# Bitcoin-Wildlife-Sanctuary/recursive-stwo

Measured on AMD Instinct MI355X. Metric: recursive proofs verified/sec, higher is better.
Workload: dtype u32 (M31 modular integers)

## Files before the change

### recursive-stwo_amd/csrc/poseidon2.hpp

```cpp
#pragma once
#include "field.hpp"

namespace rsv {

struct State16 {
    uint32_t s[16];
};

#define RSV_RC_FULL_INIT { \
    {0x768bab52, 0x70e0ab7d, 0x3d266c8a, 0x6da42045, 0x600fef22, 0x41dace6b, 0x64f9bdd4, 0x5d42d4fe, \
     0x76b1516d, 0x6fc9a717, 0x70ac4fb6, 0x00194ef6, 0x22b644e2, 0x1f7916d5, 0x47581be2, 0x2710a123}, \
    {0x6284e867, 0x018d3afe, 0x5df99ef3, 0x4c1e467b, 0x566f6abc, 0x2994e427, 0x538a6d42, 0x5d7bf2cf, \
     0x7fda2dab, 0x0fd854c4, 0x46922fca, 0x3d7763a1, 0x19fd05ca, 0x0a4bbb43, 0x15075851, 0x3d903d76}, \
    {0x2d290ff7, 0x40809fa0, 0x59dac6ec, 0x127927a2, 0x6bbf0ea0, 0x0294140f, 0x24742976, 0x6e84c081, \
     0x22484f4a, 0x354cae59, 0x0453ffe1, 0x3f47a3cc, 0x0088204e, 0x6066e109, 0x3b7c4b80, 0x6b55665d}, \
    {0x3bc4b897, 0x735bf378, 0x508daf42, 0x1884fc2b, 0x7214f24c, 0x7498be0a, 0x1a60e640, 0x3303f928, \
     0x29b46376, 0x5c96bb68, 0x65d097a5, 0x1d358e9f, 0x4a9a9017, 0x4724cf76, 0x347af70f, 0x1e77e59a}, \
    {0x57090613, 0x1fa42108, 0x17bbef50, 0x1ff7e11c, 0x047b24ca, 0x4e140275, 0x4fa086f5, 0x079b309c, \
     0x1159bd47, 0x6d37e4e5, 0x075d8dce, 0x12121ca0, 0x7f6a7c40, 0x68e182ba, 0x5493201b, 0x0444a80e}, \
    {0x0064f4c6, 0x6467abe6, 0x66975762, 0x2af68f9b, 0x345b33be, 0x1b70d47f, 0x053db717, 0x381189cb, \
     0x43b915f8, 0x20df3694, 0x0f459d26, 0x77a0e97b, 0x2f73e739, 0x1876c2f9, 0x65a0e29a, 0x4cabefbe}, \
    {0x5abd1268, 0x4d34a760, 0x12771799, 0x69a0c9ac, 0x39091e55, 0x7f611cd0, 0x3af055da, 0x7ac0bbdf, \
     0x6e0f3a24, 0x41e3b6f7, 0x49b3756d, 0x568bc538, 0x20c079d8, 0x1701c72c, 0x7670dc6c, 0x5a439035}, \
    {0x7c93e00e, 0x561fbb4d, 0x1178907b, 0x02737406, 0x32fb24f1, 0x6323b60a, 0x6ab12418, 0x42c99cea, \
     0x155a0b97, 0x53d1c6aa, 0x2bd20347, 0x279b3d73, 0x4f5f3c70, 0x0245af6c, 0x238359d3, 0x49966a59}}
__constant__ __attribute__((aligned(64))) uint32_t RC_FULL[8][16] = RSV_RC_FULL_INIT;
constexpr uint32_t RC_FULL_K[8][16] = RSV_RC_FULL_INIT;

#define RSV_RC_PARTIAL_INIT { \
   0x7f7ec4bf, 0x0421926f, 0x5198e669, 0x34db3148, 0x4368bafd, \
                                        0x66685c7f, 0x78d3249a, 0x60187881, 0x76dad67a, 0x0690b437, \
                                        0x1ea95311, 0x40e5369a, 0x38f103fc, 0x1d226a21, 0, 0}
__constant__ __attribute__((aligned(64))) uint32_t RC_PARTIAL[16] = RSV_RC_PARTIAL_INIT;
constexpr uint32_t RC_PARTIAL_K[16] = RSV_RC_PARTIAL_INIT;

__device__ __forceinline__ uint32_t pow5_ref(uint32_t x) {
    uint32_t x2 = m_sqr(x);
    return m_mul(m_sqr(x2), x);
}

__device__ __forceinline__ void mds4_ref(uint32_t& x0, uint32_t& x1, uint32_t& x2, uint32_t& x3) {
    uint32_t t0 = m_add(x0, x1), t1 = m_add(x2, x3);
    uint32_t t2 = m_add(m_dbl(x1), t1), t3 = m_add(m_dbl(x3), t0);
    uint32_t t4 = m_add(m_shl(t1, 2), t3), t5 = m_add(m_shl(t0, 2), t2);
    x0 = m_add(t3, t5);
    x1 = t5;
    x2 = m_add(t2, t4);
    x3 = t4;
}

__device__ __forceinline__ void mds16_ref(uint32_t* s) {
#pragma unroll
    for (int g = 0; g < 4; g++) mds4_ref(s[4 * g], s[4 * g + 1], s[4 * g + 2], s[4 * g + 3]);
#pragma unroll
    for (int j = 0; j < 4; j++) {
        uint32_t sum = m_add(m_add(s[j], s[j + 4]), m_add(s[j + 8], s[j + 12]));
#pragma unroll
        for (int g = 0; g < 4; g++) s[4 * g + j] = m_add(s[4 * g + j], sum);
    }
}

__device__ __forceinline__ void poseidon2_ref_inline(uint32_t* s) {
    mds16_ref(s);
#pragma unroll 1
    for (int r = 0; r < 4; r++) {
#pragma unroll
        for (int i = 0; i < 16; i++) s[i] = pow5_ref(m_add(s[i], RC_FULL[r][i]));
        mds16_ref(s);
    }
#pragma unroll 1
    for (int r = 0; r < 14; r++) {
        s[0] = pow5_ref(m_add(s[0], RC_PARTIAL[r]));
        uint32_t a0 = m_add(s[0], s[1]), a1 = m_add(s[2], s[3]), a2 = m_add(s[4], s[5]), a3 = m_add(s[6], s[7]);
        uint32_t a4 = m_add(s[8], s[9]), a5 = m_add(s[10], s[11]), a6 = m_add(s[12], s[13]),
                 a7 = m_add(s[14], s[15]);
        uint32_t sum = m_add(m_add(m_add(a0, a1), m_add(a2, a3)), m_add(m_add(a4, a5), m_add(a6, a7)));
        s[0] = m_add(sum, m_add(m_dbl(s[0]), s[0]));
#pragma unroll
        for (int i = 1; i < 16; i++) s[i] = m_add(sum, m_shl(s[i], i + 1));
    }
#pragma unroll 1
    for (int r = 4; r < 8; r++) {
#pragma unroll
        for (int i = 0; i < 16; i++) s[i] = pow5_ref(m_add(s[i], RC_FULL[r][i]));
        mds16_ref(s);
    }
}


template <bool PACE>
struct PermT {
    static __device__ __forceinline__ uint64_t add64(uint64_t a, uint64_t b) {
        uint64_t d;
        asm("v_lshl_add_u64 %0, %1, 0, %2" : "=v"(d) : "v"(a), "v"(b));
        return d;
    }
    template <int SH>
    static __device__ __forceinline__ uint64_t shl_add64(uint64_t a, uint64_t b) {
        uint64_t d;
        asm("v_lshl_add_u64 %0, %1, %3, %2" : "=v"(d) : "v"(a), "v"(b), "n"(SH));
        return d;
    }
    static __device__ __forceinline__ uint32_t opaque(uint32_t k) {
        uint32_t r;
        asm volatile("s_mov_b32 %0, %1" : "=s"(r) : "n"(k));
        return r;
    }
    static __device__ __forceinline__ uint64_t mul64(uint32_t a, uint32_t b) {
        uint64_t d, carry;
        if constexpr (PACE) asm("v_mad_u64_u32 %0, %1, %2, %3, 0\n\ts_nop 0" : "=v"(d), "=s"(carry) : "v"(a), "v"(b));
        else asm("v_mad_u64_u32 %0, %1, %2, %3, 0" : "=v"(d), "=s"(carry) : "v"(a), "v"(b));
        return d;
    }
    static __device__ __forceinline__ uint64_t mul64(uint32_t a, uint32_t b_uniform, int) {
        uint64_t d, carry;
        if constexpr (PACE) asm("v_mad_u64_u32 %0, %1, %2, %3, 0\n\ts_nop 0" : "=v"(d), "=s"(carry) : "v"(a), "s"(b_uniform));
        else asm("v_mad_u64_u32 %0, %1, %2, %3, 0" : "=v"(d), "=s"(carry) : "v"(a), "s"(b_uniform));
        return d;
    }
    static __device__ __forceinline__ uint64_t mad64(uint32_t a, uint32_t b_uniform, uint64_t c) {
        uint64_t d, carry;
        if constexpr (PACE) asm("v_mad_u64_u32 %0, %1, %2, %3, %4\n\ts_nop 0" : "=v"(d), "=s"(carry) : "v"(a), "s"(b_uniform), "v"(c));
        else asm("v_mad_u64_u32 %0, %1, %2, %3, %4" : "=v"(d), "=s"(carry) : "v"(a), "s"(b_uniform), "v"(c));
        return d;
    }
    static __device__ __forceinline__ uint32_t dbl32(uint32_t x) {
        uint32_t d;
        asm("v_add_u32 %0, %1, %1" : "=v"(d) : "v"(x));
        return d;
    }
    static __device__ __forceinline__ uint32_t fold2(uint64_t V) {
        uint32_t r = (uint32_t)(V >> 32) + ((uint32_t)V >> 1);
        return r;
    }
    static __device__ __forceinline__ uint32_t canon(uint32_t t) {
        uint32_t r = min(t, t - P);
        if constexpr (PACE) asm volatile("s_nop 0" : "+v"(r));
        return r;
    }

    static __device__ __forceinline__ uint32_t pow5(uint32_t x) {
        const uint32_t xx = dbl32(x);
        uint32_t c2 = canon(fold2(mul64(xx, x)));
        uint32_t c4 = canon(fold2(mul64(dbl32(c2), c2)));
        return fold2(mul64(xx, c4));
    }

    static __device__ __forceinline__ void mds4_2x(uint32_t k2, uint32_t k4, uint32_t x0, uint32_t x1, uint32_t x2, uint32_t x3,
                                            uint64_t& y0, uint64_t& y1, uint64_t& y2, uint64_t& y3) {
        uint64_t T0 = mad64(x0, k2, mul64(x1, k2, 0));
        uint64_t T1 = mad64(x2, k2, mul64(x3, k2, 0));
        uint64_t T2 = mad64(x1, k4, T1);
        uint64_t T3 = mad64(x3, k4, T0);
        uint64_t T4 = shl_add64<2>(T1, T3);
        uint64_t T5 = shl_add64<2>(T0, T2);
        y0 = add64(T3, T5);
        y1 = T5;
        y2 = add64(T2, T4);
        y3 = T4;
    }

    static __device__ __forceinline__ void mds16_2x(uint32_t k2, uint32_t k4, const uint32_t* s, uint64_t* V) {
    #pragma unroll
        for (int g = 0; g < 4; g++)
            mds4_2x(k2, k4, s[4 * g], s[4 * g + 1], s[4 * g + 2], s[4 * g + 3], V[4 * g], V[4 * g + 1], V[4 * g + 2], V[4 * g + 3]);
    #pragma unroll
        for (int j = 0; j < 4; j++) {
            uint64_t sum = add64(add64(V[j], V[j + 4]), add64(V[j + 8], V[j + 12]));
    #pragma unroll
            for (int g = 0; g < 4; g++) V[4 * g + j] = add64(V[4 * g + j], sum);
        }
    }

    template <uint32_t RC>
    static __device__ __forceinline__ uint32_t canon_rc(uint32_t t) {
        static_assert(RC < P - (1u << 19), "round constant too close to P for the fused reduction");
        constexpr uint32_t c = P - RC;
        uint32_t r = min(t - c, t + (P - c));
        if constexpr (PACE) asm volatile("s_nop 0" : "+v"(r));
        return r;
    }

    template <int R, int I>
    static __device__ __forceinline__ void sbox_full(const uint64_t* V, uint32_t* s) {
        s[I] = pow5(canon_rc<RC_FULL_K[R][I]>(fold2(V[I])));
        if constexpr (I + 1 < 16) sbox_full<R, I + 1>(V, s);
    }
    template <int I>
    static __device__ __forceinline__ void sbox_full4(uint32_t* s) {
        s[I] = pow5(canon_rc<RC_FULL_K[4][I]>(s[I]));
        if constexpr (I + 1 < 16) sbox_full4<I + 1>(s);
    }

    template <int R>
    static __device__ __forceinline__ void partial_round(uint32_t* s, uint32_t k2, uint32_t k6, const uint32_t* kd) {
        uint32_t u0 = pow5(canon_rc<RC_PARTIAL_K[R]>(s[0]));
        uint64_t a = mul64(u0, k2, 0), b = mul64(s[1], k2, 0);
    #pragma unroll
        for (int i = 2; i < 16; i += 2) { a = mad64(s[i], k2, a); b = mad64(s[i + 1], k2, b); }
        uint64_t sum2 = add64(a, b);
        s[0] = fold2(mad64(u0, k6, sum2));
    #pragma unroll
        for (int i = 1; i < 16; i++) s[i] = fold2(mad64(s[i], kd[i], sum2));
    }

    static __device__ __forceinline__ void poseidon2_rounds(uint32_t* s, uint32_t k2, uint32_t k4) {
        uint64_t V[16];
        const uint32_t k6 = opaque(6);
        mds16_2x(k2, k4, s, V);
        sbox_full<0, 0>(V, s); mds16_2x(k2, k4, s, V);
        sbox_full<1, 0>(V, s); mds16_2x(k2, k4, s, V);
        sbox_full<2, 0>(V, s); mds16_2x(k2, k4, s, V);
        sbox_full<3, 0>(V, s); mds16_2x(k2, k4, s, V);
    #pragma unroll
        for (int i = 0; i < 16; i++) s[i] = fold2(V[i]);
        uint32_t kd[16];
        kd[0] = k6;
    #define RSV_KD(i) kd[i] = opaque(4u << (i));
        RSV_KD(1) RSV_KD(2) RSV_KD(3) RSV_KD(4) RSV_KD(5) RSV_KD(6) RSV_KD(7) RSV_KD(8)
        RSV_KD(9) RSV_KD(10) RSV_KD(11) RSV_KD(12) RSV_KD(13) RSV_KD(14) RSV_KD(15)
    #undef RSV_KD
        partial_round<0>(s, k2, k6, kd);  partial_round<1>(s, k2, k6, kd);  partial_round<2>(s, k2, k6, kd);
        partial_round<3>(s, k2, k6, kd);  partial_round<4>(s, k2, k6, kd);  partial_round<5>(s, k2, k6, kd);
        partial_round<6>(s, k2, k6, kd);  partial_round<7>(s, k2, k6, kd);  partial_round<8>(s, k2, k6, kd);
        partial_round<9>(s, k2, k6, kd);  partial_round<10>(s, k2, k6, kd); partial_round<11>(s, k2, k6, kd);
        partial_round<12>(s, k2, k6, kd); partial_round<13>(s, k2, k6, kd);
        sbox_full4<0>(s);      mds16_2x(k2, k4, s, V);
        sbox_full<5, 0>(V, s); mds16_2x(k2, k4, s, V);
        sbox_full<6, 0>(V, s); mds16_2x(k2, k4, s, V);
        sbox_full<7, 0>(V, s);
    }

    static __device__ __forceinline__ void poseidon2_inline(uint32_t* s) {
        const uint32_t k2 = opaque(2), k4 = opaque(4);
        poseidon2_rounds(s, k2, k4);
        uint64_t V[16];
        mds16_2x(k2, k4, s, V);
    #pragma unroll
        for (int i = 0; i < 16; i++) {
            uint32_t t = fold2(V[i]);
            s[i] = min(t, t - P);
        }
    }

    template <bool HI_CONST = false, bool HI_VALUE = false>
    static __device__ __forceinline__ void poseidon2_inline_half(uint32_t* s, uint32_t hi, uint32_t* out8) {
        if (HI_CONST) hi = HI_VALUE ? 1u : 0u;
        const uint32_t k2 = opaque(2), k4 = opaque(4);
        poseidon2_rounds(s, k2, k4);
        uint64_t V[16];
    #pragma unroll
        for (int g = 0; g < 4; g++)
            mds4_2x(k2, k4, s[4 * g], s[4 * g + 1], s[4 * g + 2], s[4 * g + 3], V[4 * g], V[4 * g + 1], V[4 * g + 2], V[4 * g + 3]);
        if (hi) {
    #pragma unroll
            for (int j = 0; j < 4; j++) {
                const uint64_t sum = add64(add64(V[j], V[j + 4]), add64(V[j + 8], V[j + 12]));
                const uint32_t t0 = fold2(add64(V[8 + j], sum)), t1 = fold2(add64(V[12 + j], sum));
                out8[j] = min(t0, t0 - P);
                out8[4 + j] = min(t1, t1 - P);
            }
        } else {
    #pragma unroll
            for (int j = 0; j < 4; j++) {
                const uint64_t sum = add64(add64(V[j], V[j + 4]), add64(V[j + 8], V[j + 12]));
                const uint32_t t0 = fold2(add64(V[j], sum)), t1 = fold2(add64(V[4 + j], sum));
                out8[j] = min(t0, t0 - P);
                out8[4 + j] = min(t1, t1 - P);
            }
        }
    }
};
__device__ __forceinline__ void poseidon2_inline(uint32_t* s) { PermT<true>::poseidon2_inline(s); }

#ifdef RSV_COUNT_PERMS
__device__ unsigned long long g_perm_counter[16];
__shared__ unsigned s_perm_tag;
#define RSV_TAG(k) do { if (threadIdx.x == 0) s_perm_tag = (k); __syncthreads(); } while (0)
#else
#define RSV_TAG(k) do { } while (0)
#endif

__device__ __noinline__ State16 poseidon2(State16 st) {
#ifdef RSV_COUNT_PERMS
    {
        const unsigned long long m = __ballot(1);
        if ((threadIdx.x & 63u) == (unsigned)__builtin_ctzll(m)) {
            atomicAdd(&g_perm_counter[2 * (s_perm_tag & 7u)], (unsigned long long)__builtin_popcountll(m));
            atomicAdd(&g_perm_counter[2 * (s_perm_tag & 7u) + 1], 1ull);
        }
    }
#endif
    poseidon2_inline(st.s);
    return st;
}

struct Hash8 {
    uint32_t w[8];
};
__device__ __forceinline__ State16 join(const Hash8& l, const Hash8& r) {
    State16 st;
#pragma unroll
    for (int i = 0; i < 8; i++) { st.s[i] = l.w[i]; st.s[8 + i] = r.w[i]; }
    return st;
}
__device__ __forceinline__ Hash8 rate_of(const State16& st) {
    Hash8 h;
#pragma unroll
    for (int i = 0; i < 8; i++) h.w[i] = st.s[i];
    return h;
}
__device__ __forceinline__ Hash8 cap_of(const State16& st) {
    Hash8 h;
#pragma unroll
    for (int i = 0; i < 8; i++) h.w[i] = st.s[8 + i];
    return h;
}
__device__ __forceinline__ Hash8 zero8() {
    Hash8 h;
#pragma unroll
    for (int i = 0; i < 8; i++) h.w[i] = 0;
    return h;
}
template <bool HI, bool PACE>
__device__ __noinline__ Hash8 poseidon2_half_t(State16 st) {
#ifdef RSV_COUNT_PERMS
    {
        const unsigned long long m = __ballot(1);
        if ((threadIdx.x & 63u) == (unsigned)__builtin_ctzll(m)) {
            atomicAdd(&g_perm_counter[2 * (s_perm_tag & 7u)], (unsigned long long)__builtin_popcountll(m));
            atomicAdd(&g_perm_counter[2 * (s_perm_tag & 7u) + 1], 1ull);
        }
    }
#endif
    Hash8 h;
    PermT<PACE>::template poseidon2_inline_half<true, HI>(st.s, 0u, h.w);
    return h;
}
struct RowRC {
    uint32_t f[8];
};
__device__ __forceinline__ RowRC load_row_rc(uint32_t i) {
    RowRC k;
#pragma unroll
    for (int r = 0; r < 8; r++) k.f[r] = RC_FULL[r][i];
    return k;
}
template <bool HI>
__device__ __noinline__ Hash8 poseidon2_row_half(State16 st);
__device__ __noinline__ State16 poseidon2_row_state(State16 st);
__shared__ uint32_t s_row_rc[8][16];
template <int PACE>
__device__ __forceinline__ void row_rc_init() {
    if constexpr (PACE == 2) {
        if (threadIdx.x < 128) s_row_rc[threadIdx.x >> 4][threadIdx.x & 15u] = RC_FULL[threadIdx.x >> 4][threadIdx.x & 15u];
        __syncthreads();
    }
}
constexpr int FORM_ROW = 2;
template <int PACE = 1>
__device__ __forceinline__ Hash8 poseidon2_half(State16 st, uint32_t hi) {
    if constexpr (PACE == FORM_ROW) return hi ? poseidon2_row_half<true>(st) : poseidon2_row_half<false>(st);
    else return hi ? poseidon2_half_t<true, PACE != 0>(st) : poseidon2_half_t<false, PACE != 0>(st);
}
template <int PACE = 1>
__device__ __forceinline__ State16 poseidon2_full(State16 st) {
    if constexpr (PACE == FORM_ROW) return poseidon2_row_state(st);
    else return poseidon2(st);
}
template <int PACE>
__device__ __forceinline__ uint32_t vlane() { return PACE == FORM_ROW ? threadIdx.x >> 4 : threadIdx.x; }
template <int PACE = 1>
__device__ __forceinline__ Hash8 perm_rate(const Hash8& l, const Hash8& r) { return poseidon2_half<PACE>(join(l, r), 0u); }
template <int PACE = 1>
__device__ __forceinline__ Hash8 perm_cap(const Hash8& l, const Hash8& r) { return poseidon2_half<PACE>(join(l, r), 1u); }
__device__ __forceinline__ bool hash_eq(const Hash8& a, const Hash8& b) {
    uint32_t d = 0;
#pragma unroll
    for (int i = 0; i < 8; i++) d |= a.w[i] ^ b.w[i];
    return d == 0;
}

}
```

Before: 1.907 million.

## Fuse consecutive Poseidon2 partial rounds into algebraically merged pairs

Adds a partial_pair routine that applies two partial rounds with one set of per-lane reductions. The second round's linear layer is composed with the first, using precomputed squared diagonal constants (kq) and a correction term through the folded sum. This cuts the 64-bit fold reductions on the 15 non-sbox lanes from two per round pair to one, shortening the serial dependency chain. In exchange it needs extra constant registers, and larger intermediate magnitudes that the tightened static_assert bounds must still cover.

```diff
diff --git a/recursive-stwo_amd/csrc/poseidon2.hpp b/recursive-stwo_amd/csrc/poseidon2.hpp
--- a/recursive-stwo_amd/csrc/poseidon2.hpp
+++ b/recursive-stwo_amd/csrc/poseidon2.hpp
@@ -172,9 +172,10 @@
         }
     }
 
-    template <uint32_t RC>
+    static constexpr uint32_t HI_FULL = 160, HI_PARTIAL = 1u << 18;
+    template <uint32_t RC, uint32_t HI>
     static __device__ __forceinline__ uint32_t canon_rc(uint32_t t) {
-        static_assert(RC < P - (1u << 19), "round constant too close to P for the fused reduction");
+        static_assert(HI < P - RC, "round constant too close to P for the fused reduction");
         constexpr uint32_t c = P - RC;
         uint32_t r = min(t - c, t + (P - c));
         if constexpr (PACE) asm volatile("s_nop 0" : "+v"(r));
@@ -183,18 +184,18 @@
 
     template <int R, int I>
     static __device__ __forceinline__ void sbox_full(const uint64_t* V, uint32_t* s) {
-        s[I] = pow5(canon_rc<RC_FULL_K[R][I]>(fold2(V[I])));
+        s[I] = pow5(canon_rc<RC_FULL_K[R][I], HI_FULL>(fold2(V[I])));
         if constexpr (I + 1 < 16) sbox_full<R, I + 1>(V, s);
     }
     template <int I>
     static __device__ __forceinline__ void sbox_full4(uint32_t* s) {
-        s[I] = pow5(canon_rc<RC_FULL_K[4][I]>(s[I]));
+        s[I] = pow5(canon_rc<RC_FULL_K[4][I], HI_PARTIAL>(s[I]));
         if constexpr (I + 1 < 16) sbox_full4<I + 1>(s);
     }
 
     template <int R>
     static __device__ __forceinline__ void partial_round(uint32_t* s, uint32_t k2, uint32_t k6, const uint32_t* kd) {
-        uint32_t u0 = pow5(canon_rc<RC_PARTIAL_K[R]>(s[0]));
+        uint32_t u0 = pow5(canon_rc<RC_PARTIAL_K[R], HI_PARTIAL>(s[0]));
         uint64_t a = mul64(u0, k2, 0), b = mul64(s[1], k2, 0);
     #pragma unroll
         for (int i = 2; i < 16; i += 2) { a = mad64(s[i], k2, a); b = mad64(s[i + 1], k2, b); }
@@ -202,6 +203,27 @@
         s[0] = fold2(mad64(u0, k6, sum2));
     #pragma unroll
         for (int i = 1; i < 16; i++) s[i] = fold2(mad64(s[i], kd[i], sum2));
+    }
+
+    template <int R>
+    static __device__ __forceinline__ void partial_pair(uint32_t* s, uint32_t k2, uint32_t k6, uint32_t k30, const uint32_t* kd,
+                                                        const uint32_t* kq) {
+        uint32_t u0 = pow5(canon_rc<RC_PARTIAL_K[R], HI_PARTIAL>(s[0]));
+        uint64_t a = mul64(u0, k2, 0), b = mul64(s[1], k2, 0);
+    #pragma unroll
+        for (int i = 2; i < 16; i += 2) { a = mad64(s[i], k2, a); b = mad64(s[i + 1], k2, b); }
+        uint64_t sum2 = add64(a, b);
+        const uint32_t s0 = fold2(mad64(u0, k6, sum2));
+        const uint32_t sf = fold2(sum2);
+        u0 = pow5(canon_rc<RC_PARTIAL_K[R + 1], HI_PARTIAL>(s0));
+        a = mul64(u0, k2, 0); b = mul64(s[1], kd[1], 0);
+    #pragma unroll
+        for (int i = 2; i < 16; i += 2) { a = mad64(s[i], kd[i], a); b = mad64(s[i + 1], kd[i + 1], b); }
+        a = mad64(sf, k30, a);
+        sum2 = add64(a, b);
+        s[0] = fold2(mad64(u0, k6, sum2));
+    #pragma unroll
+        for (int i = 1; i < 16; i++) s[i] = fold2(mad64(s[i], kq[i], mad64(sf, kd[i], sum2)));
     }
 
     static __device__ __forceinline__ void poseidon2_rounds(uint32_t* s, uint32_t k2, uint32_t k4) {
@@ -220,11 +242,19 @@
         RSV_KD(1) RSV_KD(2) RSV_KD(3) RSV_KD(4) RSV_KD(5) RSV_KD(6) RSV_KD(7) RSV_KD(8)
         RSV_KD(9) RSV_KD(10) RSV_KD(11) RSV_KD(12) RSV_KD(13) RSV_KD(14) RSV_KD(15)
     #undef RSV_KD
-        partial_round<0>(s, k2, k6, kd);  partial_round<1>(s, k2, k6, kd);  partial_round<2>(s, k2, k6, kd);
-        partial_round<3>(s, k2, k6, kd);  partial_round<4>(s, k2, k6, kd);  partial_round<5>(s, k2, k6, kd);
-        partial_round<6>(s, k2, k6, kd);  partial_round<7>(s, k2, k6, kd);  partial_round<8>(s, k2, k6, kd);
-        partial_round<9>(s, k2, k6, kd);  partial_round<10>(s, k2, k6, kd); partial_round<11>(s, k2, k6, kd);
-        partial_round<12>(s, k2, k6, kd); partial_round<13>(s, k2, k6, kd);
+        uint32_t kq[16];
+        kq[0] = 0;
+    #pragma unroll
+        for (int i = 1; i < 8; i++) kq[i] = kd[2 * i + 1];
+    #define RSV_KQ(i) kq[i] = opaque(8u << (2 * (i)));
+        RSV_KQ(8) RSV_KQ(9) RSV_KQ(10) RSV_KQ(11) RSV_KQ(12) RSV_KQ(13) RSV_KQ(14)
+    #undef RSV_KQ
+        kq[15] = k4;
+        const uint32_t k30 = opaque(30);
+        partial_round<0>(s, k2, k6, kd);
+        partial_pair<1>(s, k2, k6, k30, kd, kq);  partial_pair<3>(s, k2, k6, k30, kd, kq);  partial_pair<5>(s, k2, k6, k30, kd, kq);
+        partial_pair<7>(s, k2, k6, k30, kd, kq);  partial_pair<9>(s, k2, k6, k30, kd, kq);  partial_pair<11>(s, k2, k6, k30, kd, kq);
+        partial_round<13>(s, k2, k6, kd);
         sbox_full4<0>(s);      mds16_2x(k2, k4, s, V);
         sbox_full<5, 0>(V, s); mds16_2x(k2, k4, s, V);
         sbox_full<6, 0>(V, s); mds16_2x(k2, k4, s, V);
```

Result: faster. 1.966 million, median of 6 (+3.1%).
